# egyptdj/graph-neural-mapping

Hardware: AMD Instinct MI355X
Metric: graphs/sec fwd+bwd, 400-node dense FC graphs, hidden_dim 64, 5 layers (higher is better)
Workload: dtype f32

## Files before the change

### graph-neural-mapping_amd/csrc/linear.hip

```cpp
#include "gnm_split.h"

static bool lin_force_generic() { static const bool v = getenv("GNM_LIN_GENERIC") != nullptr; return v; }
static bool lin_no_stream() { static const bool v = getenv("GNM_LIN_NO_STREAM") != nullptr; return v; }

struct LinArgs {
    const float* X;
    const float* W;
    const float* bias;
    float* Z;
    const float* pro_scale;
    const float* pro_shift;
    double* stats_partial;
    int ldx, ldw, ldz;
    int N, K, H;
    int w_kmajor;
    int pro_relu;
    unsigned long long* stamps;
    int stat_rows;
    int stage_out;
    const float* mZ; const float* m_scale; const float* m_shift; const float* m_mean; const float* m_rstd;
    int ldmz;
};

__host__ __device__ __forceinline__ int lin_first_tile_of(int wave, int groups, int rows, int nwg, int b) {
// ... 1635 lines not shown
        for (; b + 3 * ngrp < nblk; b += 4 * ngrp) {
            const float v0 = partial[(size_t)(b + 0 * ngrp) * stride + e], v1 = partial[(size_t)(b + 1 * ngrp) * stride + e];
            const float v2 = partial[(size_t)(b + 2 * ngrp) * stride + e], v3 = partial[(size_t)(b + 3 * ngrp) * stride + e];
            s0 += v0; s1 += v1; s2 += v2; s3 += v3;
        }
        for (; b < nblk; b += ngrp) s0 += partial[(size_t)b * stride + e];
    }
    red[grp][tid & 31] = (s0 + s1) + (s2 + s3);
    __syncthreads();
    float s = 0.f;
    if (tid < 32 && e < count)
        for (int g = 0; g < ngrp; ++g) s += red[g][tid];
    return s;
}

__global__ void __launch_bounds__(1024) gnm_reduce_partials_kernel(const float* __restrict__ partial, int nblk,
                                                                   long long stride, int H, int kw, int k0,
                                                                   float* __restrict__ dW, int ldw,
                                                                   float* __restrict__ db) {
    __shared__ float red[32][32];
    const int tid = threadIdx.x;
    const int e = blockIdx.x * 32 + (tid & 31);
    const int count = H * kw + H;
    const float s = reduce_partials_element(partial, nblk, stride, e, count, red);
    if (tid < 32 && e < count) {
        if (e < H * kw) {
            const int row = e / kw, col = e - row * kw;
            dW[(size_t)row * ldw + k0 + col] = s;
        } else if (db && k0 == 0) {
            db[e - H * kw] = s;
        }
    }
}

static int launch_reduce_partials(const float* workspace, int nblk, int H, int kw, int k0, float* dW, int ldw, float* db,
                                  hipStream_t s) {
    const long long stride = (long long)H * kw + H;
    const int count = H * kw + H;
    hipLaunchKernelGGL(gnm_reduce_partials_kernel, dim3((count + 31) / 32), dim3(1024), 0, s, workspace, nblk, stride,
                       H, kw, k0, dW, ldw, db);
    GNM_CHECK_LAUNCH();
    return GNM_OK;
}

struct LbArgs {
    const float* G; const float* Z; const float* X; const float* W;
    const float* mean; const float* rstd; const float* cA; const float* m1; const float* m2;
    const float* pro_scale; const float* pro_shift;
    float* dA; float* partial;
    const float* sZ; const float* s_scale; const float* s_shift; const float* s_mean; const float* s_rstd;
    double* s_partial;
    int ldg, ldz, ldx, ldw, lda, ldsz;
    int N, K, H;
    int pro_relu;
    unsigned long long* stamps;
    const float* bias;
    int part_rows;
};

static inline LbArgs lb_args(const float* G, int ldg, const float* mean, const float* rstd, const float* cA,
                             const float* m1, const float* m2, const float* X, int ldx, const float* pro_scale,
                             const float* pro_shift, int pro_relu, const float* W, int ldw, float* dA, int lda,
                             float* workspace, int N, int K, int H, const float* sZ, int ldsz, const float* s_scale,
                             const float* s_shift, const float* s_mean, const float* s_rstd, double* s_partial) {
    LbArgs a = {};
    a.sZ = sZ; a.s_scale = s_scale; a.s_shift = s_shift; a.s_mean = s_mean; a.s_rstd = s_rstd;
    a.s_partial = s_partial; a.ldsz = ldsz;
    a.G = G; a.X = X; a.W = W; a.mean = mean; a.rstd = rstd; a.cA = cA; a.m1 = m1; a.m2 = m2;
    a.pro_scale = pro_scale; a.pro_shift = pro_shift; a.dA = dA; a.partial = workspace;
    a.ldg = ldg; a.ldx = ldx; a.ldw = ldw; a.lda = lda; a.N = N; a.K = K; a.H = H; a.pro_relu = pro_relu;
    a.stamps = g_lin_stamps;
    return a;
}

constexpr size_t lb_dump_bytes(int HT, int KT, int NW) { return ((size_t)NW * HT * KT * 1024 + (size_t)NW * HT * 64) * 4; }
template <int KT, int HT, bool SPLITD, bool COEF>
struct LbLds {
    static constexpr int KP = KT * 32, HP = HT * 32, XS = (KP > HP ? KP : HP) + 4, EW = 4 * KT * 64;
    static constexpr size_t xs_off = SPLITD ? (size_t)3 * EW * 16 : (size_t)HP * KP * 4;
    static constexpr size_t coef_off = xs_off + (size_t)4 * 32 * XS * 4;
    static constexpr size_t body = coef_off + (COEF ? (size_t)5 * HP * 4 : 0);
    static constexpr size_t total = body > lb_dump_bytes(HT, KT, 4) ? body : lb_dump_bytes(HT, KT, 4);
    static_assert((size_t)4 * 2 * KP * 8 <= body, "the lower BatchNorm's sums [4][2][KP] fp64 reuse the body");
};
static constexpr int kRzWaves = 8;
template <bool NARROW>
struct RzLds {
    static constexpr int EWF = NARROW ? 128 : 512, EWB = NARROW ? 256 : 512, XS = 68, KT = NARROW ? 1 : 2;
    static constexpr size_t wb_off = (size_t)3 * EWF * 16;
    static constexpr size_t xs_off = wb_off + (size_t)3 * EWB * 16;
    static constexpr size_t coef_off = xs_off + (size_t)kRzWaves * 32 * XS * 4;
    static constexpr size_t psv_off = coef_off + (size_t)6 * 64 * 4;
    static constexpr size_t body = psv_off + (NARROW ? 0 : (size_t)2 * 64 * 4);
    static constexpr size_t total = body > lb_dump_bytes(2, KT, kRzWaves) ? body : lb_dump_bytes(2, KT, kRzWaves);
};

template <int HP, bool BIAS>
__device__ __forceinline__ void lb_stage_coef(float* coef, const float* mean, const float* rstd, const float* cA,
                                              const float* m1, const float* m2, const float* bias, int tid, int nt) {
    for (int idx = tid; idx < HP; idx += nt) {
        coef[idx] = mean[idx]; coef[HP + idx] = rstd[idx]; coef[2 * HP + idx] = cA[idx];
        coef[3 * HP + idx] = m1[idx]; coef[4 * HP + idx] = m2[idx];
        if (BIAS) coef[5 * HP + idx] = bias ? bias[idx] : 0.f;
    }
}

template <int HT, int KT, int GROUPS, bool CLIP>
__device__ __forceinline__ void lb_combine(char* smem, const f32x16 (&wacc)[HT][KT], const float (&dbacc)[HT], float* partial,
                                           int H, int K, int part_rows, int tid, int lane, int wave) {
    constexpr int TILE = 16 * 64, WT = HT * KT * TILE, NW = 4 * GROUPS, NT = NW * 64;
    __syncthreads();
    float* dump = reinterpret_cast<float*>(smem);
    float* mine = dump + (size_t)wave * WT;
#pragma unroll
    for (int a = 0; a < HT; ++a)
#pragma unroll
        for (int b = 0; b < KT; ++b)
#pragma unroll
            for (int r = 0; r < 16; ++r) mine[(a * KT + b) * TILE + r * 64 + lane] = wacc[a][b][r];
    float* dbdump = dump + (size_t)NW * WT;
#pragma unroll
    for (int a = 0; a < HT; ++a) dbdump[(wave * HT + a) * 64 + lane] = dbacc[a];
    __syncthreads();
    const size_t pstride = (size_t)H * K + H;
    for (int idx = tid; idx < GROUPS * WT; idx += NT) {
        const int grp = idx / WT, rem = idx - grp * WT;
        const int prow = blockIdx.x * GROUPS + grp;
        if (GROUPS > 1 && prow >= part_rows) continue;
        const int ab = rem / TILE;
        const int rl = rem - ab * TILE;
        const int r = rl >> 6, ln = rl & 63;
        const int a = ab / KT, b = ab - a * KT;
        const int row = 32 * a + (r & 3) + 8 * (r >> 2) + 4 * (ln >> 5);
        const int col = 32 * b + (ln & 31);
        if (CLIP && col >= K) continue;
        float sum = 0.f;
#pragma unroll
        for (int w = 0; w < 4; ++w) sum += dump[(size_t)(4 * grp + w) * WT + rem];
        partial[(size_t)prow * pstride + (size_t)row * K + col] = sum;
    }
    for (int idx = tid; idx < GROUPS * HT * 32; idx += NT) {
        const int grp = idx / (HT * 32), a = (idx >> 5) % HT, ii = idx & 31;
        const int prow = blockIdx.x * GROUPS + grp;
        if (GROUPS > 1 && prow >= part_rows) continue;
        float sum = 0.f;
#pragma unroll
        for (int w = 0; w < 4; ++w) sum += dbdump[((4 * grp + w) * HT + a) * 64 + ii] + dbdump[((4 * grp + w) * HT + a) * 64 + 32 + ii];
        partial[(size_t)prow * pstride + (size_t)H * K + 32 * a + ii] = sum;
    }
}

template <int KT, int HT, bool STATS, bool NARROW = false, bool SAMEZ = false, bool SPLITD = false>
__global__ void __launch_bounds__(256, 2) gnm_linear_bwd_fused_kernel(const LbArgs p) {
    static_assert(!SPLITD || (HT == 2 && ((SAMEZ && KT == 2) || NARROW)), "SPLITD: H = 64, the SAMEZ K = 64 form or the narrow one");
    static_assert(!NARROW || (KT == 1 && !STATS), "narrow K: one tile, no lower BatchNorm");
    static_assert(!SAMEZ || STATS, "SAMEZ is a STATS variant");
    using L = LbLds<KT, HT, SPLITD, false>;
    constexpr int KP = L::KP, HP = L::HP, XS = L::XS, EW = L::EW;
    constexpr int H4 = HP / 4;
    constexpr int NLD = (32 * H4) / 64;
    constexpr int RSTEP = 64 / H4;
    constexpr int KH = HP / 2;
    constexpr int O4 = KP / 4;
    extern __shared__ __attribute__((aligned(16))) char smem[];
    float* Wt = reinterpret_cast<float*>(smem);
    gnm_u32x4* Wp = reinterpret_cast<gnm_u32x4*>(smem);
    float* Xs_all = reinterpret_cast<float*>(smem + L::xs_off);
    const int tid = threadIdx.x;
    const int lane = tid & 63;
    const int wave = __builtin_amdgcn_readfirstlane(tid >> 6);
    const int i = lane & 31, h = lane >> 5;
    float* Xs = Xs_all + wave * 32 * XS;
    GNM_LSTAMP(0)
    if constexpr (SPLITD) {
        for (int e = tid; e < EW; e += 256) {
            const int n = e & 31, kg = (e >> 5) & 1, c = (e >> 6) % KT, m = e / (64 * KT);
            float f[8];
#pragma unroll
            for (int j = 0; j < 8; ++j)
                f[j] = (!NARROW || 32 * c + n < p.K) ? p.W[(size_t)(8 * m + 32 * kg + j) * p.ldw + 32 * c + n] : 0.f;
            gnm_u32x4 p1, p2, p3;
            gnm_split8(f, p1, p2, p3);
            Wp[e] = p1; Wp[EW + e] = p2; Wp[2 * EW + e] = p3;
        }
    } else {
        for (int idx = tid; idx < HP * KP; idx += 256) {
            const int hh = idx / KP, k = idx - hh * KP;
            Wt[idx] = (!NARROW || k < p.K) ? p.W[(size_t)hh * p.ldw + k] : 0.f;
        }
    }
    __syncthreads();
    GNM_LSTAMP(1)
    int tk = 0;

    const int c4 = lane % H4, lrow0 = lane / H4;
    float4 mu, rs, ca, a1, a2;
    if constexpr (!SAMEZ) {
        mu = *reinterpret_cast<const float4*>(p.mean + 4 * c4);
        rs = *reinterpret_cast<const float4*>(p.rstd + 4 * c4);
        ca = *reinterpret_cast<const float4*>(p.cA + 4 * c4);
        a1 = *reinterpret_cast<const float4*>(p.m1 + 4 * c4);
        a2 = *reinterpret_cast<const float4*>(p.m2 + 4 * c4);
    }
    float psc[KT], psh[KT];
#pragma unroll
    for (int b = 0; b < KT; ++b) {
        const bool kin = !NARROW || 32 * b + i < p.K;
        psc[b] = (p.pro_scale && kin) ? p.pro_scale[32 * b + i] : 1.f;
        psh[b] = (p.pro_scale && kin) ? p.pro_shift[32 * b + i] : 0.f;
    }
    f32x16 wacc[HT][KT];
#pragma unroll
    for (int a = 0; a < HT; ++a)
#pragma unroll
        for (int b = 0; b < KT; ++b)
#pragma unroll
            for (int r = 0; r < 16; ++r) wacc[a][b][r] = 0.f;
    float dbacc[HT];
#pragma unroll
    for (int a = 0; a < HT; ++a) dbacc[a] = 0.f;
    constexpr int OR = 64 / O4;
    const int oc4 = lane % O4, orow0 = lane / O4;
    float4 ss1 = make_float4(0.f, 0.f, 0.f, 0.f), ss2 = ss1;
    float cmu[KT], crs[KT], cs1[KT], cs2[KT];
#pragma unroll
    for (int b = 0; b < KT; ++b) {
        cmu[b] = SAMEZ ? p.s_mean[32 * b + i] : 0.f;
        crs[b] = SAMEZ ? p.s_rstd[32 * b + i] : 0.f;
        cs1[b] = 0.f; cs2[b] = 0.f;
    }

    const int ntiles = (p.N + 31) / 32;
    const int nlast = p.N - 1;
    for (int t = lin_first_tile(wave, 1, gridDim.x); t < ntiles; t += gridDim.x * 4) {
        const int r0 = t * 32;
        GNM_LSTAMP(2 + 5 * min(tk, 11))
        float4 g4[NLD], z4[NLD];
#pragma unroll
        for (int j = 0; j < NLD; ++j) {
            const int grow = min(r0 + lrow0 + j * RSTEP, nlast);
            g4[j] = *reinterpret_cast<const float4*>(p.G + (size_t)grow * p.ldg + 4 * c4);
            z4[j] = *reinterpret_cast<const float4*>(p.Z + (size_t)grow * p.ldz + 4 * c4);
        }
        if constexpr (SAMEZ) {
            mu = *reinterpret_cast<const float4*>(p.mean + 4 * c4);
            rs = *reinterpret_cast<const float4*>(p.rstd + 4 * c4);
            ca = *reinterpret_cast<const float4*>(p.cA + 4 * c4);
            a1 = *reinterpret_cast<const float4*>(p.m1 + 4 * c4);
            a2 = *reinterpret_cast<const float4*>(p.m2 + 4 * c4);
        }
        __builtin_amdgcn_sched_barrier(0);
#pragma unroll
        for (int j = 0; j < NLD; ++j) {
            const int lrow = lrow0 + j * RSTEP;
            float4 d;
            d.x = ca.x * (g4[j].x - a1.x - (z4[j].x - mu.x) * rs.x * a2.x);
            d.y = ca.y * (g4[j].y - a1.y - (z4[j].y - mu.y) * rs.y * a2.y);
            d.z = ca.z * (g4[j].z - a1.z - (z4[j].z - mu.z) * rs.z * a2.z);
            d.w = ca.w * (g4[j].w - a1.w - (z4[j].w - mu.w) * rs.w * a2.w);
            if (r0 + lrow >= p.N) d = make_float4(0.f, 0.f, 0.f, 0.f);
            *reinterpret_cast<float4*>(Xs + lrow * XS + 4 * c4) = d;
        }
        __builtin_amdgcn_fence(__ATOMIC_RELEASE, "wavefront");
        __builtin_amdgcn_wave_barrier();
        __builtin_amdgcn_fence(__ATOMIC_ACQUIRE, "wavefront");
        float xv[16][KT];
#pragma unroll
        for (int s = 0; s < 16; ++s) {
            const int krow = SAMEZ ? (s & 3) + 8 * (s >> 2) + 4 * h : 2 * s + h;
            const int grow = min(r0 + krow, nlast);
#pragma unroll
            for (int b = 0; b < KT; ++b)
                xv[s][b] = (!NARROW || 32 * b + i < p.K) ? p.X[(size_t)grow * p.ldx + 32 * b + i] : 0.f;
        }
        __builtin_amdgcn_sched_barrier(0);
        GNM_LSTAMP(3 + 5 * min(tk, 11))
        f32x16 dacc[KT];
        if constexpr (SPLITD) {
            if (p.dA) {
#pragma unroll
                for (int c = 0; c < KT; ++c)
#pragma unroll
                    for (int r = 0; r < 16; ++r) dacc[c][r] = 0.f;
                lin_dgrad_split<KT, HP>(dacc, Xs, XS, Wp, i, h, lane);
            }
        } else if (p.dA) {
            float a[KH];
#pragma unroll
            for (int j = 0; j < KH / 4; ++j) {
                const float4 v = *reinterpret_cast<const float4*>(Xs + i * XS + KH * h + 4 * j);
                a[4 * j + 0] = v.x; a[4 * j + 1] = v.y; a[4 * j + 2] = v.z; a[4 * j + 3] = v.w;
            }
#pragma unroll
            for (int c = 0; c < KT; ++c)
#pragma unroll
                for (int r = 0; r < 16; ++r) dacc[c][r] = 0.f;
            const float* wrow = Wt + (size_t)(KH * h) * KP + i;
#pragma unroll
            for (int s = 0; s < KH; ++s) {
#pragma unroll
                for (int c = 0; c < KT; ++c)
                    dacc[c] = __builtin_amdgcn_mfma_f32_32x32x2f32(a[s], wrow[s * KP + 32 * c], dacc[c], 0, 0, 0);
            }
        }
        GNM_LSTAMP(4 + 5 * min(tk, 11))
#pragma unroll
        for (int s = 0; s < 16; ++s) {
// ... 188 lines not shown
#pragma unroll
            for (int r = 0; r < 16; ++r) wacc[a][b][r] = 0.f;
    float dbacc[HT];
#pragma unroll
    for (int a = 0; a < HT; ++a) dbacc[a] = 0.f;

    const int ntiles = (p.N + 31) / 32;
    const int tstride = gridDim.x * 4;
    const int gz_voff_g = (lrow0 * p.ldg + 4 * c4) * 4, gz_step_g = RSTEP * p.ldg * 4;
    const int gz_voff_z = (lrow0 * p.ldz + 4 * c4) * 4, gz_step_z = RSTEP * p.ldz * 4;
    const int x_voff = (h * p.ldx + i) * 4;
    const int out_voff = ((lane / O4) * p.lda + 4 * (lane % O4)) * 4, out_step = (64 / O4) * p.lda * 4;
    const float* dxbase = p.dA ? p.dA : p.G;

    gnm_u32x4 g4[NLD], z4[NLD];
    auto load_gz = [&](int tile) {
        const long long row0 = (long long)tile * 32;
        const long long rows = min((long long)p.N - row0, 32LL);
        const __amdgpu_buffer_rsrc_t rg = gnm_tile_rsrc(p.G + row0 * p.ldg, rows, p.ldg, HP);
        const __amdgpu_buffer_rsrc_t rz = gnm_tile_rsrc(p.Z + row0 * p.ldz, rows, p.ldz, HP);
#pragma unroll
        for (int j = 0; j < NLD; ++j) {
            g4[j] = __builtin_amdgcn_raw_buffer_load_b128(rg, gz_voff_g, j * gz_step_g, 0);
            z4[j] = __builtin_amdgcn_raw_buffer_load_b128(rz, gz_voff_z, j * gz_step_z, 0);
        }
    };
    auto do_tile = [&](int t, int t_next) {
        const int r0 = t * 32;
        const int rows = min(p.N - r0, 32);
        const float4 mu = *reinterpret_cast<const float4*>(coef + 4 * c4);
        const float4 rs = *reinterpret_cast<const float4*>(coef + HP + 4 * c4);
        const float4 ca = *reinterpret_cast<const float4*>(coef + 2 * HP + 4 * c4);
        const float4 a1 = *reinterpret_cast<const float4*>(coef + 3 * HP + 4 * c4);
        const float4 a2 = *reinterpret_cast<const float4*>(coef + 4 * HP + 4 * c4);
#pragma unroll
        for (int j = 0; j < NLD; ++j) {
            const int lrow = lrow0 + j * RSTEP;
            const float4 gj = __builtin_bit_cast(float4, g4[j]), zj = __builtin_bit_cast(float4, z4[j]);
            float4 d;
            d.x = ca.x * (gj.x - a1.x - (zj.x - mu.x) * rs.x * a2.x);
            d.y = ca.y * (gj.y - a1.y - (zj.y - mu.y) * rs.y * a2.y);
            d.z = ca.z * (gj.z - a1.z - (zj.z - mu.z) * rs.z * a2.z);
            d.w = ca.w * (gj.w - a1.w - (zj.w - mu.w) * rs.w * a2.w);
            if (lrow >= rows) d = make_float4(0.f, 0.f, 0.f, 0.f);
            *reinterpret_cast<float4*>(Xs + lrow * XS + 4 * c4) = d;
        }
        __builtin_amdgcn_fence(__ATOMIC_RELEASE, "wavefront");
        __builtin_amdgcn_wave_barrier();
        __builtin_amdgcn_fence(__ATOMIC_ACQUIRE, "wavefront");
        float xv[16][KT];
        {
            const __amdgpu_buffer_rsrc_t rx = gnm_tile_rsrc(p.X + (size_t)r0 * p.ldx, rows, p.ldx, KP);
#pragma unroll
            for (int s = 0; s < 16; ++s)
#pragma unroll
                for (int b = 0; b < KT; ++b)
                    xv[s][b] = __uint_as_float(__builtin_amdgcn_raw_buffer_load_b32(rx, x_voff, (2 * s * p.ldx + 32 * b) * 4, 0));
        }
        __builtin_amdgcn_sched_barrier(0);
        f32x16 dacc[KT];
        if constexpr (SPLITD) {
#pragma unroll
            for (int c = 0; c < KT; ++c)
#pragma unroll
                for (int r = 0; r < 16; ++r) dacc[c][r] = 0.f;
            lin_dgrad_split<KT, HP>(dacc, Xs, XS, Wp, i, h, lane);
        } else {
            float a[KH];
#pragma unroll
            for (int j = 0; j < KH / 4; ++j) {
                const float4 v = *reinterpret_cast<const float4*>(Xs + i * XS + KH * h + 4 * j);
                a[4 * j + 0] = v.x; a[4 * j + 1] = v.y; a[4 * j + 2] = v.z; a[4 * j + 3] = v.w;
            }
#pragma unroll
            for (int c = 0; c < KT; ++c)
#pragma unroll
                for (int r = 0; r < 16; ++r) dacc[c][r] = 0.f;
            const float* wrow = Wt + (size_t)(KH * h) * KP + i;
#pragma unroll
            for (int s = 0; s < KH; ++s) {
#pragma unroll
                for (int c = 0; c < KT; ++c)
                    dacc[c] = __builtin_amdgcn_mfma_f32_32x32x2f32(a[s], wrow[s * KP + 32 * c], dacc[c], 0, 0, 0);
            }
        }
        load_gz(t_next);
#pragma unroll
        for (int s = 0; s < 16; ++s) {
            float av[HT];
            const int krow = 2 * s + h;
#pragma unroll
            for (int a = 0; a < HT; ++a) av[a] = Xs[krow * XS + 32 * a + i];
            float xf[KT];
#pragma unroll
            for (int b = 0; b < KT; ++b) {
                float x = xv[s][b];
                if (p.pro_scale) {
                    x = x * psc[b] + psh[b];
                    if (p.pro_relu) x = gnm_relu(x);
                }
                xf[b] = x;
            }
#pragma unroll
            for (int a = 0; a < HT; ++a) {
                dbacc[a] += av[a];
#pragma unroll
                for (int b = 0; b < KT; ++b)
                    wacc[a][b] = __builtin_amdgcn_mfma_f32_32x32x2f32(av[a], xf[b], wacc[a][b], 0, 0, 0);
            }
        }
        __builtin_amdgcn_fence(__ATOMIC_RELEASE, "wavefront");
        __builtin_amdgcn_wave_barrier();
#pragma unroll
        for (int c = 0; c < KT; ++c)
#pragma unroll
            for (int r = 0; r < 16; ++r) Xs[((r & 3) + 8 * (r >> 2) + 4 * h) * XS + 32 * c + i] = dacc[c][r];
        __builtin_amdgcn_fence(__ATOMIC_RELEASE, "wavefront");
        __builtin_amdgcn_wave_barrier();
        __builtin_amdgcn_fence(__ATOMIC_ACQUIRE, "wavefront");
        {
            const __amdgpu_buffer_rsrc_t rd = gnm_tile_rsrc(dxbase + (p.dA ? (size_t)r0 * p.lda : 0), p.dA ? rows : 0, p.lda, KP);
#pragma unroll
            for (int st = 0; st < (32 * O4) / 64; ++st) {
                const int idx = lane + 64 * st;
                const int row = idx / O4, oc = idx - row * O4;
                const gnm_u32x4 v = *reinterpret_cast<const gnm_u32x4*>(Xs + row * XS + 4 * oc);
                __builtin_amdgcn_raw_buffer_store_b128(v, rd, out_voff + st * out_step, 0, 0);
            }
        }
        __builtin_amdgcn_fence(__ATOMIC_RELEASE, "wavefront");
        __builtin_amdgcn_wave_barrier();
    };
    {
        int t = lin_first_tile(wave, 1, gridDim.x);
        load_gz(t);
        if (t < ntiles) {
            do_tile(t, t + tstride);
            for (t += tstride; t < ntiles; t += tstride) do_tile(t, t + tstride);
        }
    }

    lb_combine<HT, KT, 1, false>(smem, wacc, dbacc, p.partial, p.H, p.K, 0, tid, lane, wave);
}

template <int KT, int HT, bool SPLITD = false>
static int launch_lb_pipe(const LbArgs& a, int grid, hipStream_t s) {
    const size_t lds = LbLds<KT, HT, SPLITD, true>::total;
    GNM_ALLOW_FULL_LDS((&gnm_linear_bwd_pipe_kernel<KT, HT, SPLITD>));
    hipLaunchKernelGGL((gnm_linear_bwd_pipe_kernel<KT, HT, SPLITD>), dim3(grid), dim3(256), lds, s, a);
    GNM_CHECK_LAUNCH();
    return GNM_OK;
}

template <int KT, int HT, bool STATS, bool NARROW = false, bool SAMEZ = false, bool SPLITD = false>
static int launch_lb(const LbArgs& a, int grid, hipStream_t s) {
    const size_t lds = LbLds<KT, HT, SPLITD, false>::total;
    GNM_ALLOW_FULL_LDS((&gnm_linear_bwd_fused_kernel<KT, HT, STATS, NARROW, SAMEZ, SPLITD>));
    hipLaunchKernelGGL((gnm_linear_bwd_fused_kernel<KT, HT, STATS, NARROW, SAMEZ, SPLITD>), dim3(grid), dim3(256), lds, s, a);
    GNM_CHECK_LAUNCH();
    return GNM_OK;
}

__device__ __forceinline__ void rz_load_g(float (&g)[2][16], const float* G, int ldg, int N, int tile, int g_voff) {
    const long long row0 = (long long)tile * 32;
    const long long rows = min((long long)N - row0, 32LL);
    const __amdgpu_buffer_rsrc_t rg = gnm_tile_rsrc(G + row0 * ldg, rows, ldg, 64);
#pragma unroll
    for (int r = 0; r < 16; ++r)
#pragma unroll
        for (int a = 0; a < 2; ++a)
            g[a][r] = __uint_as_float(__builtin_amdgcn_raw_buffer_load_b32(rg, g_voff + 128 * a, ((r & 3) + 8 * (r >> 2)) * ldg * 4, 0));
}
__device__ __forceinline__ float rz_bn_bwd(f32x16& dz, const float (&g)[16], const float* coef, int col, int rows, float* Xs,
                                           int xs, int h) {
    const float mu = coef[col], rs = coef[64 + col], ca = coef[128 + col], a1 = coef[192 + col], a2 = coef[256 + col],
                bz = coef[320 + col];
    float dsum = 0.f;
#pragma unroll
    for (int r = 0; r < 16; ++r) {
        const int lrow = (r & 3) + 8 * (r >> 2) + 4 * h;
        const float z = dz[r] + bz;
        float d = ca * (g[r] - a1 - (z - mu) * rs * a2);
        if (lrow >= rows) d = 0.f;
        dz[r] = d;
        dsum += d;
        Xs[lrow * xs + col] = d;
    }
    return dsum;
}

__global__ void __launch_bounds__(kRzWaves * 64) gnm_linear_bwd_rz_kernel(const LbArgs p) {
    using L = RzLds<false>;
    constexpr int KP = 64, HP = 64, XS = L::XS, EW = 512, NW = kRzWaves, NT = NW * 64;
    static_assert(L::EWF == EW && L::EWB == EW, "both plane images hold 4 m x 2 c x 64 entries");
    extern __shared__ __attribute__((aligned(16))) char smem[];
    gnm_u32x4* Wf = reinterpret_cast<gnm_u32x4*>(smem);
    gnm_u32x4* Wb = reinterpret_cast<gnm_u32x4*>(smem + L::wb_off);
    float* Xs_all = reinterpret_cast<float*>(smem + L::xs_off);
    float* coef = reinterpret_cast<float*>(smem + L::coef_off);
    float* psv = reinterpret_cast<float*>(smem + L::psv_off);
    const int tid = threadIdx.x;
    const int lane = tid & 63;
    const int wave = __builtin_amdgcn_readfirstlane(tid >> 6);
    const int i = lane & 31, h = lane >> 5;
    float* Xs = Xs_all + wave * 32 * XS;
    const bool pro = p.pro_scale != nullptr;
    GNM_RSTAMP(0)
    lin_stage_planes<2, 32, false, false>(Wf, EW, p.W, p.ldw, 0, tid, NT);
    lin_stage_planes<2, 32, true, false>(Wb, EW, p.W, p.ldw, 0, tid, NT);
    lb_stage_coef<64, true>(coef, p.mean, p.rstd, p.cA, p.m1, p.m2, p.bias, tid, NT);
    for (int idx = tid; idx < 64; idx += NT) {
        psv[idx] = pro ? p.pro_scale[idx] : 1.f;
        psv[64 + idx] = pro ? p.pro_shift[idx] : 0.f;
    }
    float psc[2], psh[2];
#pragma unroll
    for (int b = 0; b < 2; ++b) {
        psc[b] = pro ? p.pro_scale[32 * b + i] : 1.f;
        psh[b] = pro ? p.pro_shift[32 * b + i] : 0.f;
    }
    __builtin_amdgcn_s_waitcnt(0x0F70);
    __syncthreads();
    GNM_RSTAMP(1)
    int tk = 0;

    f32x16 wacc[2][2];
#pragma unroll
    for (int a = 0; a < 2; ++a)
#pragma unroll
        for (int b = 0; b < 2; ++b)
#pragma unroll
            for (int r = 0; r < 16; ++r) wacc[a][b][r] = 0.f;
    float dbacc[2] = {0.f, 0.f};

    const int gw = lin_first_tile(wave, NW / 4, p.part_rows);
    const int ntiles = (p.N + 31) / 32;
    const int tstride = p.part_rows * 4;
    const int g_voff = (4 * h * p.ldg + i) * 4;
    const int xa_voff = (i * p.ldx + 32 * h) * 4;
    const int xc_voff = (4 * h * p.ldx + i) * 4;
    const int out_voff = ((lane >> 4) * p.lda + 4 * (lane & 15)) * 4, out_step = 4 * p.lda * 4;

    float g[2][16];
    gnm_u32x4 xa[4][2];
    auto load_next_x = [&](int tile) {
        const long long row0 = (long long)tile * 32;
        const long long rows = min((long long)p.N - row0, 32LL);
        const __amdgpu_buffer_rsrc_t rx = gnm_tile_rsrc(p.X + row0 * p.ldx, rows, p.ldx, KP);
#pragma unroll
        for (int m = 0; m < 4; ++m) {
            xa[m][0] = __builtin_amdgcn_raw_buffer_load_b128(rx, xa_voff, 32 * m, 0);
            xa[m][1] = __builtin_amdgcn_raw_buffer_load_b128(rx, xa_voff, 32 * m + 16, 0);
        }
    };
    auto do_tile = [&](int t, int t_next) {
        const int r0 = t * 32;
        const int rows = min(p.N - r0, 32);
        GNM_RSTAMP(2 + 6 * min(tk, 9))
        f32x16 dz[2];
#pragma unroll
        for (int c = 0; c < 2; ++c)
#pragma unroll
            for (int r = 0; r < 16; ++r) dz[c][r] = 0.f;
#pragma unroll
        for (int m = 0; m < 4; ++m) {
            const float4 v0 = __builtin_bit_cast(float4, xa[m][0]), v1 = __builtin_bit_cast(float4, xa[m][1]);
            float f[8] = {v0.x, v0.y, v0.z, v0.w, v1.x, v1.y, v1.z, v1.w};
            if (pro) {
                const int k0 = 32 * h + 8 * m;
#pragma unroll
                for (int q = 0; q < 2; ++q) {
                    const float4 sc = *reinterpret_cast<const float4*>(psv + k0 + 4 * q);
                    const float4 sh = *reinterpret_cast<const float4*>(psv + 64 + k0 + 4 * q);
                    f[4 * q + 0] = f[4 * q + 0] * sc.x + sh.x; f[4 * q + 1] = f[4 * q + 1] * sc.y + sh.y;
                    f[4 * q + 2] = f[4 * q + 2] * sc.z + sh.z; f[4 * q + 3] = f[4 * q + 3] * sc.w + sh.w;
                }
                if (p.pro_relu) {
#pragma unroll
                    for (int j = 0; j < 8; ++j) f[j] = gnm_relu(f[j]);
                }
            }
            gnm_bf16x8 a1, a2, a3;
            gnm_split8(f, a1, a2, a3);
#pragma unroll
            for (int c = 0; c < 2; ++c) gnm_mma6_planes(dz[c], a1, a2, a3, Wf, EW, (m * 2 + c) * 64 + lane);
        }
        GNM_RSTAMP(3 + 6 * min(tk, 9))
#pragma unroll
        for (int a = 0; a < 2; ++a) dbacc[a] += rz_bn_bwd(dz[a], g[a], coef, 32 * a + i, rows, Xs, XS, h);
        __builtin_amdgcn_fence(__ATOMIC_RELEASE, "wavefront");
        __builtin_amdgcn_wave_barrier();
        __builtin_amdgcn_fence(__ATOMIC_ACQUIRE, "wavefront");
        float xv[16][2];
        {
            const __amdgpu_buffer_rsrc_t rx = gnm_tile_rsrc(p.X + (size_t)r0 * p.ldx, rows, p.ldx, KP);
#pragma unroll
            for (int r = 0; r < 16; ++r)
#pragma unroll
                for (int b = 0; b < 2; ++b)
                    xv[r][b] = __uint_as_float(__builtin_amdgcn_raw_buffer_load_b32(rx, xc_voff + 128 * b, ((r & 3) + 8 * (r >> 2)) * p.ldx * 4, 0));
        }
        __builtin_amdgcn_sched_barrier(0);
        GNM_RSTAMP(4 + 6 * min(tk, 9))
        f32x16 dacc[2];
#pragma unroll
        for (int c = 0; c < 2; ++c)
// ... 129 lines not shown
#pragma unroll
        for (int c = 0; c < 2; ++c)
#pragma unroll
            for (int r = 0; r < 16; ++r) dz[c][r] = 0.f;
        {
            gnm_bf16x8 a1, a2, a3;
            gnm_split8(fx, a1, a2, a3);
#pragma unroll
            for (int c = 0; c < 2; ++c) gnm_mma6_planes(dz[c], a1, a2, a3, Wf, L::EWF, c * 64 + lane);
        }
#pragma unroll
        for (int a = 0; a < 2; ++a) dbacc[a] += rz_bn_bwd(dz[a], g[a], coef, 32 * a + i, rows, Xs, XS, h);
        __builtin_amdgcn_fence(__ATOMIC_RELEASE, "wavefront");
        __builtin_amdgcn_wave_barrier();
        __builtin_amdgcn_fence(__ATOMIC_ACQUIRE, "wavefront");
        if (p.dA) {
            f32x16 dacc[1];
#pragma unroll
            for (int r = 0; r < 16; ++r) dacc[0][r] = 0.f;
            lin_dgrad_split<1, HP>(dacc, Xs, XS, Wb, i, h, lane);
            const __amdgpu_buffer_rsrc_t rd = gnm_tile_rsrc(p.dA + (size_t)r0 * p.lda, rows, p.lda, K);
#pragma unroll
            for (int r = 0; r < 16; ++r)
                __builtin_amdgcn_raw_buffer_store_b32(__float_as_uint(dacc[0][r]), rd, da_voff, ((r & 3) + 8 * (r >> 2)) * p.lda * 4, 0);
        }
        __builtin_amdgcn_fence(__ATOMIC_RELEASE, "wavefront");
        __builtin_amdgcn_wave_barrier();
        rz_load_g(g, p.G, p.ldg, p.N, t_next, (int)g_voff);
#pragma unroll
        for (int m = 0; m < 2; ++m) {
            float f[8];
            gnm_bf16x8 x1, x2, x3, d1, d2, d3;
#pragma unroll
            for (int j = 0; j < 8; ++j) f[j] = xv[8 * m + j];
            gnm_split8(f, x1, x2, x3);
#pragma unroll
            for (int a = 0; a < 2; ++a) {
#pragma unroll
                for (int j = 0; j < 8; ++j) f[j] = dz[a][8 * m + j];
                gnm_split8(f, d1, d2, d3);
                gnm_mma6(wacc[a], d1, d2, d3, x1, x2, x3);
            }
        }
    };
    {
        int t = gw;
        rz_load_g(g, p.G, p.ldg, p.N, t, (int)g_voff);
        if (t < ntiles) {
            do_tile(t, t + tstride);
            for (t += tstride; t < ntiles; t += tstride) do_tile(t, t + tstride);
        }
    }
    __builtin_amdgcn_s_waitcnt(0x0F70);
    __syncthreads();
    float* dump = reinterpret_cast<float*>(smem);
    float* mine = dump + (size_t)wave * 2 * TILE;
#pragma unroll
    for (int a = 0; a < 2; ++a)
#pragma unroll
        for (int r = 0; r < 16; ++r) mine[a * TILE + r * 64 + lane] = wacc[a][r];
    float* dbdump = dump + (size_t)NW * 2 * TILE;
#pragma unroll
    for (int a = 0; a < 2; ++a) dbdump[(wave * 2 + a) * 64 + lane] = dbacc[a];
    __syncthreads();
    const size_t pstride = (size_t)HP * K + HP;
    for (int idx = tid; idx < 2 * 2 * TILE; idx += NT) {
        const int grp = idx / (2 * TILE), rem = idx - grp * 2 * TILE;
        const int prow = blockIdx.x * 2 + grp;
        if (prow >= p.part_rows) continue;
        const int a = rem / TILE;
        const int rl = rem - a * TILE;
        const int r = rl >> 6, ln = rl & 63;
        const int row = 32 * a + (r & 3) + 8 * (r >> 2) + 4 * (ln >> 5);
        const int col = ln & 31;
        if (col >= K) continue;
        float sum = 0.f;
#pragma unroll
        for (int w = 0; w < 4; ++w) sum += dump[(size_t)(4 * grp + w) * 2 * TILE + rem];
        p.partial[(size_t)prow * pstride + (size_t)row * K + col] = sum;
    }
    for (int idx = tid; idx < 2 * 64; idx += NT) {
        const int grp = idx >> 6, a = (idx >> 5) & 1, ii = idx & 31;
        const int prow = blockIdx.x * 2 + grp;
        if (prow >= p.part_rows) continue;
        float sum = 0.f;
#pragma unroll
        for (int w = 0; w < 4; ++w) sum += dbdump[((4 * grp + w) * 2 + a) * 64 + ii] + dbdump[((4 * grp + w) * 2 + a) * 64 + 32 + ii];
        p.partial[(size_t)prow * pstride + (size_t)HP * K + 32 * a + ii] = sum;
    }
}

static int launch_lb_rzn(const LbArgs& a, int grid, hipStream_t s) {
    const size_t lds = RzLds<true>::total;
    GNM_ALLOW_FULL_LDS((&gnm_linear_bwd_rzn_kernel));
    hipLaunchKernelGGL(gnm_linear_bwd_rzn_kernel, dim3((grid + 1) / 2), dim3(kRzWaves * 64), lds, s, a);
    GNM_CHECK_LAUNCH();
    return GNM_OK;
}

extern "C" int gnm_linear_bwd_grid(int N) {
    int g = ((N + 31) / 32 + 3) / 4;
    static const int cap = gnm_env_int("GNM_LINBWD_GRID", 512);
    if (g > cap) g = cap;
    return g < 1 ? 1 : g;
}
extern "C" long long gnm_linear_bwd_workspace_floats(int N, int H, int K) {
    return (long long)gnm_linear_bwd_grid(N) * ((long long)H * K + H);
}

extern "C" int gnm_linear_bwd_fused(const float* G, int ldg, const float* Z, int ldz, const float* mean,
                                    const float* rstd, const float* cA, const float* m1, const float* m2,
                                    const float* X, int ldx, const float* pro_scale, const float* pro_shift,
                                    int pro_relu, const float* W, int ldw, float* dA, int lda, float* dW, int lddw,
                                    float* db, float* workspace, int N, int K, int H, const float* sZ, int ldsz,
                                    const float* s_scale, const float* s_shift, const float* s_mean,
                                    const float* s_rstd, double* s_partial, void* stream) {
    if (N <= 0) return GNM_ERR_UNSUPPORTED;
    const bool narrow = K >= 1 && K < 32 && !sZ;
    if ((K != 32 && K != 64 && !narrow) || (H != 32 && H != 64)) return GNM_ERR_UNSUPPORTED;
    if ((ldg & 3) || (ldz & 3) || (dA && !narrow && (lda & 3)) || lin_force_generic()) return GNM_ERR_UNSUPPORTED;
    const uintptr_t al = reinterpret_cast<uintptr_t>(G) | reinterpret_cast<uintptr_t>(Z) |
                         (narrow ? 0 : reinterpret_cast<uintptr_t>(dA)) | reinterpret_cast<uintptr_t>(mean) |
                         reinterpret_cast<uintptr_t>(rstd) | reinterpret_cast<uintptr_t>(cA) |
                         reinterpret_cast<uintptr_t>(m1) | reinterpret_cast<uintptr_t>(m2);
    if (al & 15) return GNM_ERR_UNSUPPORTED;
    if (sZ) {
        if (!dA || !s_partial || (ldsz & 3)) return GNM_ERR_BAD_ARG;
        const uintptr_t al2 = reinterpret_cast<uintptr_t>(sZ) | reinterpret_cast<uintptr_t>(s_scale) |
                              reinterpret_cast<uintptr_t>(s_shift) | reinterpret_cast<uintptr_t>(s_mean) |
                              reinterpret_cast<uintptr_t>(s_rstd);
        if (al2 & 15) return GNM_ERR_UNSUPPORTED;
    }
    LbArgs a = lb_args(G, ldg, mean, rstd, cA, m1, m2, X, ldx, pro_scale, pro_shift, pro_relu, W, ldw, dA, lda, workspace,
                       N, K, H, sZ, ldsz, s_scale, s_shift, s_mean, s_rstd, s_partial);
    a.Z = Z; a.ldz = ldz;
    hipStream_t s = reinterpret_cast<hipStream_t>(stream);
    const int grid = gnm_linear_bwd_grid(N);
    int rc = GNM_ERR_UNSUPPORTED;
    const int KT = narrow ? 0 : K / 32, HT = H / 32;
    if (!narrow && !sZ) {
        if (KT == 1 && HT == 1) rc = launch_lb_pipe<1, 1>(a, grid, s);
        if (KT == 2 && HT == 1) rc = launch_lb_pipe<2, 1>(a, grid, s);
        if (KT == 1 && HT == 2) rc = launch_lb_pipe<1, 2>(a, grid, s);
        if (KT == 2 && HT == 2) rc = lin_no_split() ? launch_lb_pipe<2, 2>(a, grid, s) : launch_lb_pipe<2, 2, true>(a, grid, s);
    }
    if (narrow && HT == 1) rc = launch_lb<1, 1, false, true>(a, grid, s);
    if (narrow && HT == 2)
        rc = lin_no_split() ? launch_lb<1, 2, false, true>(a, grid, s) : launch_lb<1, 2, false, true, false, true>(a, grid, s);
    if (sZ && KT == 1 && HT == 1) rc = launch_lb<1, 1, true>(a, grid, s);
    if (sZ && KT == 2 && HT == 1) rc = launch_lb<2, 1, true>(a, grid, s);
    if (sZ && KT == 1 && HT == 2) rc = launch_lb<1, 2, true>(a, grid, s);
    const bool samez = sZ && sZ == X && ldsz == ldx && s_scale == pro_scale && s_shift == pro_shift && pro_relu;
    if (sZ && KT == 2 && HT == 2)
        rc = samez ? (lin_no_split() ? launch_lb<2, 2, true, false, true>(a, grid, s)
                                     : launch_lb<2, 2, true, false, true, true>(a, grid, s))
                   : launch_lb<2, 2, true>(a, grid, s);
    if (rc != GNM_OK || !dW) return rc;
    return launch_reduce_partials(workspace, grid, H, K, 0, dW, lddw, db, s);
}

extern "C" int gnm_linear_bwd_fused_rz(const float* G, int ldg, const float* bias, const float* mean, const float* rstd,
                                       const float* cA, const float* m1, const float* m2, const float* X, int ldx,
                                       const float* pro_scale, const float* pro_shift, int pro_relu, const float* W,
                                       int ldw, float* dA, int lda, float* dW, int lddw, float* db, float* workspace,
                                       int N, int K, int H, const float* sZ, int ldsz, const float* s_scale,
                                       const float* s_shift, const float* s_mean, const float* s_rstd,
                                       double* s_partial, void* stream) {
    if (sZ) return GNM_ERR_UNSUPPORTED;
    const bool narrow = K >= 1 && K <= 16 && !pro_scale;
    if (N <= 0 || (K != 64 && !narrow) || H != 64 || (!dA && !narrow) || lin_force_generic() || lin_no_split())
        return GNM_ERR_UNSUPPORTED;
    if (!narrow && ((ldx & 3) || (lda & 3))) return GNM_ERR_UNSUPPORTED;
    if (!narrow && ((reinterpret_cast<uintptr_t>(X) | reinterpret_cast<uintptr_t>(dA)) & 15)) return GNM_ERR_UNSUPPORTED;
    if ((long long)32 * (ldg > ldx ? (ldg > lda ? ldg : lda) : (ldx > lda ? ldx : lda)) * 4 >= (1LL << 31)) return GNM_ERR_UNSUPPORTED;
    LbArgs a = lb_args(G, ldg, mean, rstd, cA, m1, m2, X, ldx, pro_scale, pro_shift, pro_relu, W, ldw, dA, lda, workspace,
                       N, K, H, sZ, ldsz, s_scale, s_shift, s_mean, s_rstd, s_partial);
    hipStream_t s = reinterpret_cast<hipStream_t>(stream);
    const int grid = gnm_linear_bwd_grid(N);
    a.bias = bias; a.part_rows = grid;
    const int rc = narrow ? launch_lb_rzn(a, grid, s) : launch_lb_rz(a, grid, s);
    if (rc != GNM_OK || !dW) return rc;
    return launch_reduce_partials(workspace, grid, H, K, 0, dW, lddw, db, s);
}

#define GNM_MAX_REDUCE_JOBS 32
struct ReduceJobs {
    const float* partial[GNM_MAX_REDUCE_JOBS];
    float* dW[GNM_MAX_REDUCE_JOBS];
    float* db[GNM_MAX_REDUCE_JOBS];
    int nblk[GNM_MAX_REDUCE_JOBS], H[GNM_MAX_REDUCE_JOBS], K[GNM_MAX_REDUCE_JOBS], ldw[GNM_MAX_REDUCE_JOBS];
    int first_block[GNM_MAX_REDUCE_JOBS + 1];
    int njobs;
};
__global__ void __launch_bounds__(1024) gnm_reduce_partials_multi_kernel(const ReduceJobs J) {
    __shared__ float red[32][32];
    int j = 0;
    while (j + 1 < J.njobs && (int)blockIdx.x >= J.first_block[j + 1]) ++j;
    const float* __restrict__ partial = J.partial[j];
    const int nblk = J.nblk[j], H = J.H[j], kw = J.K[j];
    const long long stride = (long long)H * kw + H;
    const int tid = threadIdx.x;
    const int e = ((int)blockIdx.x - J.first_block[j]) * 32 + (tid & 31);
    const int count = H * kw + H;
    const float s = reduce_partials_element(partial, nblk, stride, e, count, red);
    if (tid < 32 && e < count) {
        if (e < H * kw) {
            const int row = e / kw, col = e - row * kw;
            J.dW[j][(size_t)row * J.ldw[j] + col] = s;
        } else if (J.db[j]) {
            J.db[j][e - H * kw] = s;
        }
    }
}

extern "C" int gnm_reduce_partials_multi(const float* const* workspaces_host, float* const* dW_host, const int* lddw_host,
                                         float* const* db_host, const int* Hs_host, const int* Ks_host, int njobs, int N,
                                         void* stream) {
    if (njobs <= 0) return GNM_OK;
    if (njobs > GNM_MAX_REDUCE_JOBS || N <= 0) return GNM_ERR_BAD_ARG;
    ReduceJobs J;
    int blocks = 0;
    for (int i = 0; i < njobs; ++i) {
        if (!workspaces_host[i] || !dW_host[i] || Hs_host[i] <= 0 || Ks_host[i] <= 0) return GNM_ERR_BAD_ARG;
        J.partial[i] = workspaces_host[i]; J.dW[i] = dW_host[i]; J.db[i] = db_host[i];
        J.nblk[i] = gnm_linear_bwd_grid(N); J.H[i] = Hs_host[i]; J.K[i] = Ks_host[i]; J.ldw[i] = lddw_host[i];
        J.first_block[i] = blocks;
        blocks += (Hs_host[i] * Ks_host[i] + Hs_host[i] + 31) / 32;
    }
    J.first_block[njobs] = blocks;
    J.njobs = njobs;
    hipLaunchKernelGGL(gnm_reduce_partials_multi_kernel, dim3(blocks), dim3(1024), 0, reinterpret_cast<hipStream_t>(stream), J);
    GNM_CHECK_LAUNCH();
    return GNM_OK;
}

extern "C" int gnm_linear_wgrad(const float* dZ, int ldd, const float* X, int ldx, int N, int H, int K,
                                const float* pro_scale, const float* pro_shift, int pro_relu, float* dW, int ldw,
                                float* db, float* workspace, void* stream) {
    if (H <= 0 || K <= 0 || H > 128) return GNM_ERR_BAD_ARG;
    hipStream_t s = reinterpret_cast<hipStream_t>(stream);
    const int grid = gnm_wgrad_grid(N > 0 ? N : 1);
    int rpb = ((N > 0 ? N : 1) + grid - 1) / grid;
    rpb = (rpb + 1) & ~1;
    const int HT = (H + 31) / 32;
    for (int k0 = 0; k0 < K; k0 += 128) {
        const int kw = (K - k0) < 128 ? (K - k0) : 128;
        const int KT = (kw + 31) / 32;
        WgArgs a;
        a.dZ = dZ; a.X = X; a.pro_scale = pro_scale; a.pro_shift = pro_shift; a.partial = workspace;
        a.ldd = ldd; a.ldx = ldx; a.N = N; a.H = H; a.K = K; a.k0 = k0; a.kw = kw; a.rows_per_block = rpb;
        a.pro_relu = pro_relu;
        const int WI = HT < 2 ? HT : 2, WJ = KT < 2 ? KT : 2;
        const int QI = (HT + WI - 1) / WI, QJ = (KT + WJ - 1) / WJ;
        int rc = GNM_ERR_UNSUPPORTED;
        const bool fast = (H % 32) == 0 && N > 0 && !lin_force_generic();
        if (fast && H == 128 && kw == 128 && !lin_no_split() && (long long)(rpb + 64) * (ldd > ldx ? ldd : ldx) * 4 < (1LL << 31)) {
            rc = launch_wgrad_split128(a, grid, s);
            if (rc != GNM_OK) return rc;
        } else {
#define GNM_WG_CASE(WI_, WJ_, QI_, QJ_)                                                       \
    if (WI == WI_ && WJ == WJ_ && QI == QI_ && QJ == QJ_)                                     \
        rc = fast ? launch_wgrad_fast<WI_, WJ_, QI_, QJ_>(a, grid, s) : launch_wgrad<WI_, WJ_, QI_, QJ_>(a, grid, s);
        GNM_WG_CASE(1, 1, 1, 1) GNM_WG_CASE(1, 2, 1, 1) GNM_WG_CASE(1, 2, 1, 2)
        GNM_WG_CASE(2, 1, 1, 1) GNM_WG_CASE(2, 2, 1, 1) GNM_WG_CASE(2, 2, 1, 2)
        GNM_WG_CASE(2, 1, 2, 1) GNM_WG_CASE(2, 2, 2, 1) GNM_WG_CASE(2, 2, 2, 2)
#undef GNM_WG_CASE
        }
        if (rc == GNM_OK) rc = launch_reduce_partials(workspace, grid, H, kw, k0, dW, ldw, db, s);
        if (rc != GNM_OK) return rc;
    }
    return GNM_OK;
}
```

Baseline: 419,200.

## Add pipelined backward linear kernel for the same-Z BatchNorm-stats K=64 path

Adds a dedicated pipelined kernel for the linear backward case where the lower BatchNorm input equals X (SAMEZ, K=H=64). It prefetches the next tile's G and Z via buffer loads while the current tile's dgrad, ReLU masking, stat accumulation and weight-gradient MFMAs run. The dA output is staged through a separate LDS half-buffer and written with 128-bit stores. The old SPLITD SAMEZ variant of the fused kernel is removed. This costs more LDS per workgroup and more live registers, which may limit occupancy.

```diff
diff --git a/graph-neural-mapping_amd/csrc/linear.hip b/graph-neural-mapping_amd/csrc/linear.hip
--- a/graph-neural-mapping_amd/csrc/linear.hip
+++ b/graph-neural-mapping_amd/csrc/linear.hip
@@ -1811,7 +1811,7 @@
 
 template <int KT, int HT, bool STATS, bool NARROW = false, bool SAMEZ = false, bool SPLITD = false>
 __global__ void __launch_bounds__(256, 2) gnm_linear_bwd_fused_kernel(const LbArgs p) {
-    static_assert(!SPLITD || (HT == 2 && ((SAMEZ && KT == 2) || NARROW)), "SPLITD: H = 64, the SAMEZ K = 64 form or the narrow one");
+    static_assert(!SPLITD || (HT == 2 && NARROW), "SPLITD: H = 64, the narrow form (SAMEZ K = 64: gnm_linear_bwd_pipe_sz_kernel)");
     static_assert(!NARROW || (KT == 1 && !STATS), "narrow K: one tile, no lower BatchNorm");
     static_assert(!SAMEZ || STATS, "SAMEZ is a STATS variant");
     using L = LbLds<KT, HT, SPLITD, false>;
@@ -2306,6 +2306,222 @@
     return GNM_OK;
 }
 
+struct LbSzLds {
+    using L = LbLds<2, 2, true, true>;
+    static constexpr size_t half_off = L::body;
+    static constexpr size_t body = L::body + (size_t)4 * 16 * L::XS * 4;
+    static constexpr size_t total = body > lb_dump_bytes(2, 2, 4) ? body : lb_dump_bytes(2, 2, 4);
+    static_assert(total <= 80 * 1024, "two workgroups share a CU");
+};
+__global__ void __launch_bounds__(256, 2) gnm_linear_bwd_pipe_sz_kernel(const LbArgs p) {
+    constexpr int KT = 2, HT = 2;
+    using L = LbLds<KT, HT, true, true>;
+    constexpr int KP = L::KP, HP = L::HP, XS = L::XS, EW = L::EW;
+    constexpr int H4 = HP / 4;
+    constexpr int NLD = (32 * H4) / 64;
+    constexpr int RSTEP = 64 / H4;
+    constexpr int O4 = KP / 4;
+    extern __shared__ __attribute__((aligned(16))) char smem[];
+    gnm_u32x4* Wp = reinterpret_cast<gnm_u32x4*>(smem);
+    float* Xs_all = reinterpret_cast<float*>(smem + L::xs_off);
+    float* coef = reinterpret_cast<float*>(smem + L::coef_off);
+    const int tid = threadIdx.x;
+    const int lane = tid & 63;
+    const int wave = __builtin_amdgcn_readfirstlane(tid >> 6);
+    const int i = lane & 31, h = lane >> 5;
+    float* Xs = Xs_all + wave * 32 * XS;
+    float* Hs = reinterpret_cast<float*>(smem + LbSzLds::half_off) + wave * 16 * XS;
+    lin_stage_planes<KT, 32, true, false>(Wp, EW, p.W, p.ldw, 0, tid, 256);
+    lb_stage_coef<HP, false>(coef, p.mean, p.rstd, p.cA, p.m1, p.m2, nullptr, tid, 256);
+    const int c4 = lane % H4, lrow0 = lane / H4;
+    float psc[KT], psh[KT], cmu[KT], crs[KT], cs1[KT], cs2[KT];
+#pragma unroll
+    for (int b = 0; b < KT; ++b) {
+        psc[b] = p.pro_scale ? p.pro_scale[32 * b + i] : 1.f;
+        psh[b] = p.pro_scale ? p.pro_shift[32 * b + i] : 0.f;
+        cmu[b] = p.s_mean[32 * b + i];
+        crs[b] = p.s_rstd[32 * b + i];
+        cs1[b] = 0.f; cs2[b] = 0.f;
+    }
+    __builtin_amdgcn_s_waitcnt(0x0F70);
+    __syncthreads();
+    f32x16 wacc[HT][KT];
+#pragma unroll
+    for (int a = 0; a < HT; ++a)
+#pragma unroll
+        for (int b = 0; b < KT; ++b)
+#pragma unroll
+            for (int r = 0; r < 16; ++r) wacc[a][b][r] = 0.f;
+    float dbacc[HT];
+#pragma unroll
+    for (int a = 0; a < HT; ++a) dbacc[a] = 0.f;
+
+    const int ntiles = (p.N + 31) / 32;
+    const int tstride = gridDim.x * 4;
+    const int gz_voff_g = (lrow0 * p.ldg + 4 * c4) * 4, gz_step_g = RSTEP * p.ldg * 4;
+    const int gz_voff_z = (lrow0 * p.ldz + 4 * c4) * 4, gz_step_z = RSTEP * p.ldz * 4;
+    const int x_voff = (4 * h * p.ldx + i) * 4;
+    const int out_voff = ((lane / O4) * p.lda + 4 * (lane % O4)) * 4;
+
+    gnm_u32x4 g4[NLD], z4[NLD];
+    auto load_gz = [&](int tile) {
+        const long long row0 = (long long)tile * 32;
+        const long long rows = min((long long)p.N - row0, 32LL);
+        const __amdgpu_buffer_rsrc_t rg = gnm_tile_rsrc(p.G + row0 * p.ldg, rows, p.ldg, HP);
+        const __amdgpu_buffer_rsrc_t rz = gnm_tile_rsrc(p.Z + row0 * p.ldz, rows, p.ldz, HP);
+#pragma unroll
+        for (int j = 0; j < NLD; ++j) {
+            g4[j] = __builtin_amdgcn_raw_buffer_load_b128(rg, gz_voff_g, j * gz_step_g, 0);
+            z4[j] = __builtin_amdgcn_raw_buffer_load_b128(rz, gz_voff_z, j * gz_step_z, 0);
+        }
+    };
+    auto do_tile = [&](int t, int t_next) {
+        const int r0 = t * 32;
+        const int rows = min(p.N - r0, 32);
+        const float4 mu = *reinterpret_cast<const float4*>(coef + 4 * c4);
+        const float4 rs = *reinterpret_cast<const float4*>(coef + HP + 4 * c4);
+        const float4 ca = *reinterpret_cast<const float4*>(coef + 2 * HP + 4 * c4);
+        const float4 a1 = *reinterpret_cast<const float4*>(coef + 3 * HP + 4 * c4);
+        const float4 a2 = *reinterpret_cast<const float4*>(coef + 4 * HP + 4 * c4);
+#pragma unroll
+        for (int j = 0; j < NLD; ++j) {
+            const int lrow = lrow0 + j * RSTEP;
+            const float4 gj = __builtin_bit_cast(float4, g4[j]), zj = __builtin_bit_cast(float4, z4[j]);
+            float4 d;
+            d.x = ca.x * (gj.x - a1.x - (zj.x - mu.x) * rs.x * a2.x);
+            d.y = ca.y * (gj.y - a1.y - (zj.y - mu.y) * rs.y * a2.y);
+            d.z = ca.z * (gj.z - a1.z - (zj.z - mu.z) * rs.z * a2.z);
+            d.w = ca.w * (gj.w - a1.w - (zj.w - mu.w) * rs.w * a2.w);
+            if (lrow >= rows) d = make_float4(0.f, 0.f, 0.f, 0.f);
+            *reinterpret_cast<float4*>(Xs + lrow * XS + 4 * c4) = d;
+        }
+        __builtin_amdgcn_fence(__ATOMIC_RELEASE, "wavefront");
+        __builtin_amdgcn_wave_barrier();
+        __builtin_amdgcn_fence(__ATOMIC_ACQUIRE, "wavefront");
+        float xv[16][KT];
+        {
+            const __amdgpu_buffer_rsrc_t rx = gnm_tile_rsrc(p.X + (size_t)r0 * p.ldx, rows, p.ldx, KP);
+#pragma unroll
+            for (int s = 0; s < 16; ++s)
+#pragma unroll
+                for (int b = 0; b < KT; ++b)
+                    xv[s][b] = __uint_as_float(__builtin_amdgcn_raw_buffer_load_b32(
+                        rx, x_voff, (((s & 3) + 8 * (s >> 2)) * p.ldx + 32 * b) * 4, 0));
+        }
+        __builtin_amdgcn_sched_barrier(0);
+        f32x16 dacc[KT];
+#pragma unroll
+        for (int c = 0; c < KT; ++c)
+#pragma unroll
+            for (int r = 0; r < 16; ++r) dacc[c][r] = 0.f;
+        lin_dgrad_split<KT, HP>(dacc, Xs, XS, Wp, i, h, lane);
+        {
+            const __amdgpu_buffer_rsrc_t rd = gnm_tile_rsrc(p.dA + (size_t)r0 * p.lda, rows, p.lda, KP);
+            auto mask_sum = [&](int c, int r) {
+                const float z = xv[r][c];
+                float g = dacc[c][r];
+                if (z * psc[c] + psh[c] <= 0.f) g = 0.f;
+                if ((r & 3) + 8 * (r >> 2) + 4 * h < rows) {
+                    cs1[c] += g;
+                    cs2[c] += g * ((z - cmu[c]) * crs[c]);
+                }
+                return g;
+            };
+#pragma unroll
+            for (int q = 0; q < 2; ++q) {
+                float gq[KT][8];
+#pragma unroll
+                for (int c = 0; c < KT; ++c)
+#pragma unroll
+                    for (int r = 0; r < 8; ++r) gq[c][r] = mask_sum(c, 8 * q + r);
+#pragma unroll
+                for (int c = 0; c < KT; ++c)
+#pragma unroll
+                    for (int r = 0; r < 8; ++r) Hs[((r & 3) + 8 * (r >> 2) + 4 * h) * XS + 32 * c + i] = gq[c][r];
+                __builtin_amdgcn_fence(__ATOMIC_RELEASE, "wavefront");
+                __builtin_amdgcn_wave_barrier();
+                __builtin_amdgcn_fence(__ATOMIC_ACQUIRE, "wavefront");
+#pragma unroll
+                for (int st = 0; st < (16 * O4) / 64; ++st) {
+                    const int idx = lane + 64 * st;
+                    const int row = idx / O4, oc = idx - row * O4;
+                    const gnm_u32x4 v = *reinterpret_cast<const gnm_u32x4*>(Hs + row * XS + 4 * oc);
+                    __builtin_amdgcn_raw_buffer_store_b128(v, rd, out_voff + (16 * q + (64 / O4) * st) * p.lda * 4, 0, 0);
+                }
+                __builtin_amdgcn_fence(__ATOMIC_RELEASE, "wavefront");
+                __builtin_amdgcn_wave_barrier();
+            }
+        }
+        __builtin_amdgcn_sched_barrier(0);
+        load_gz(t_next);
+        __builtin_amdgcn_sched_barrier(0);
+#pragma unroll
+        for (int s = 0; s < 16; ++s) {
+            float av[HT];
+            const int krow = (s & 3) + 8 * (s >> 2) + 4 * h;
+#pragma unroll
+            for (int a = 0; a < HT; ++a) av[a] = Xs[krow * XS + 32 * a + i];
+            float xf[KT];
+#pragma unroll
+            for (int b = 0; b < KT; ++b) {
+                float x = xv[s][b];
+                if (p.pro_scale) {
+                    x = x * psc[b] + psh[b];
+                    if (p.pro_relu) x = gnm_relu(x);
+                }
+                xf[b] = x;
+            }
+#pragma unroll
+            for (int a = 0; a < HT; ++a) {
+                dbacc[a] += av[a];
+#pragma unroll
+                for (int b = 0; b < KT; ++b)
+                    wacc[a][b] = __builtin_amdgcn_mfma_f32_32x32x2f32(av[a], xf[b], wacc[a][b], 0, 0, 0);
+            }
+        }
+        __builtin_amdgcn_fence(__ATOMIC_RELEASE, "wavefront");
+        __builtin_amdgcn_wave_barrier();
+    };
+    {
+        int t = lin_first_tile(wave, 1, gridDim.x);
+        load_gz(t);
+        if (t < ntiles) {
+            do_tile(t, t + tstride);
+            for (t += tstride; t < ntiles; t += tstride) do_tile(t, t + tstride);
+        }
+    }
+
+    __syncthreads();
+    double* sred = reinterpret_cast<double*>(smem);
+#pragma unroll
+    for (int c = 0; c < KT; ++c) {
+        double d1 = (double)cs1[c], d2 = (double)cs2[c];
+        d1 += __shfl_xor(d1, 32, 64);
+        d2 += __shfl_xor(d2, 32, 64);
+        if (h == 0) {
+            sred[(wave * 2 + 0) * KP + 32 * c + i] = d1;
+            sred[(wave * 2 + 1) * KP + 32 * c + i] = d2;
+        }
+    }
+    __syncthreads();
+    for (int idx = tid; idx < 2 * KP; idx += 256) {
+        const int which = idx / KP, col = idx - which * KP;
+        double sum = 0.0;
+        for (int w = 0; w < 4; ++w) sum += sred[(w * 2 + which) * KP + col];
+        p.s_partial[((size_t)blockIdx.x * 2 + which) * p.K + col] = sum;
+    }
+
+    lb_combine<HT, KT, 1, false>(smem, wacc, dbacc, p.partial, p.H, p.K, 0, tid, lane, wave);
+}
+
+static int launch_lb_pipe_sz(const LbArgs& a, int grid, hipStream_t s) {
+    const size_t lds = LbSzLds::total;
+    GNM_ALLOW_FULL_LDS((&gnm_linear_bwd_pipe_sz_kernel));
+    hipLaunchKernelGGL(gnm_linear_bwd_pipe_sz_kernel, dim3(grid), dim3(256), lds, s, a);
+    GNM_CHECK_LAUNCH();
+    return GNM_OK;
+}
+
 template <int KT, int HT, bool STATS, bool NARROW = false, bool SAMEZ = false, bool SPLITD = false>
 static int launch_lb(const LbArgs& a, int grid, hipStream_t s) {
     const size_t lds = LbLds<KT, HT, SPLITD, false>::total;
@@ -2741,8 +2957,7 @@
     if (sZ && KT == 1 && HT == 2) rc = launch_lb<1, 2, true>(a, grid, s);
     const bool samez = sZ && sZ == X && ldsz == ldx && s_scale == pro_scale && s_shift == pro_shift && pro_relu;
     if (sZ && KT == 2 && HT == 2)
-        rc = samez ? (lin_no_split() ? launch_lb<2, 2, true, false, true>(a, grid, s)
-                                     : launch_lb<2, 2, true, false, true, true>(a, grid, s))
+        rc = samez ? (lin_no_split() ? launch_lb<2, 2, true, false, true>(a, grid, s) : launch_lb_pipe_sz(a, grid, s))
                    : launch_lb<2, 2, true>(a, grid, s);
     if (rc != GNM_OK || !dW) return rc;
     return launch_reduce_partials(workspace, grid, H, K, 0, dW, lddw, db, s);
```

New measurement: 425,000, median of 6. 1.01x the previous value.
